# LonglongaaaGo/VSPBFR

Hardware: AMD Instinct MI355X
Metric: restored 512x512 faces/sec (higher is better)
Workload: dtype f32; 1 GPU; restoration_test.py hot path A+B+C+D, batch 8/GPU, 512x512, 50-step DDPM CodeDiffuser + StyleGAN2 prior + RestoreNet forward, fp32, random-init weights; batch_per_gpu=8, with_style_sample=True, sampler=ddpm, overlap=A+B of batch i+1 on a second HIP stream under C+D of batch i, launch=eager (one host launch per kernel)

## Files before the change

### include/vspbfr_hip.h

```cpp
#ifndef VSPBFR_HIP_H
#define VSPBFR_HIP_H

#include <stdint.h>

#ifdef __cplusplus
extern "C" {
#endif

#define VSP_ABI_VERSION 4

#define VSP_OK 0
#define VSP_EINVAL (-1)
#define VSP_ELAUNCH (-2)
#define VSP_ENOTSUP (-3)

typedef void* vsp_stream_t;

int vsp_abi_version(void);
const char* vsp_last_error(void);
int vsp_device_count(void);
int vsp_struct_size(int which);

int vsp_fused_bias_act_f32(float* out, const float* x, const float* bias, const float* ref, int64_t n,
                           int step_b, int size_b, int act, int grad, float alpha, float scale,
// ... 92 lines not shown
  const float* Bm;
  float* C;
  int Z, M, N, K;
  int64_t a_zs, a_ms, a_ks;
  int64_t b_zs, b_ns, b_ks;
  int64_t c_zs, c_ms;
  float alpha;
  const float* bias;
  float bias_scale;
  int act;
  float slope, gain;
  int64_t bias_zs;
} vsp_gemm_params;

int vsp_gemm_f32(const vsp_gemm_params* p, vsp_stream_t stream);

int vsp_pixelnorm_dim1_f32(float* out, const float* x, int Z, int R, int C, float eps, vsp_stream_t stream);
int vsp_layernorm_f32(float* out, const float* x, const float* add, const float* gamma, const float* beta,
                      int rows, int cols, float eps, int post, float slope, float gain, vsp_stream_t stream);
int vsp_softmax_lastdim_f32(float* out, const float* x, int rows, int cols, vsp_stream_t stream);
int vsp_softmax_dim1_f32(float* out, const float* x, int Z, int R, int C, vsp_stream_t stream);
int vsp_film_f32(float* out, const float* h, const float* gamma, const float* beta, int64_t n,
                 vsp_stream_t stream);
int vsp_axpby_idx_f32(float* out, const float* x, const float* y, const float* a, const float* b, int idx,
                      int64_t n, vsp_stream_t stream);
int vsp_demod_f32(float* out, const float* style, const float* wsq, int B, int Cin, int Cout, float wscale,
                  float eps, vsp_stream_t stream);
typedef struct {
  const float* w;
  const float* bias;
  const float* wsq;
  float* mod;
  float* demod;
  int64_t src_off;
  int cin, cout;
  float alpha, bias_scale, wscale2;
  int pad_;
} vsp_style_layer;
int vsp_style_plan_f32(const vsp_style_layer* table, int L, const float* src, int B, int64_t bstride, int K, int max_cin, int max_cout,
                       float eps, vsp_stream_t stream);
int vsp_demod_weight_f32(float* out, float* wsq, const float* style, const float* w, int B, int Cin, int Cout, int K, float wscale,
                         float eps, vsp_stream_t stream);
int vsp_demod_weight_bwd_f32(float* dstyle, float* dw, const float* g, const float* out, const float* style, const float* wsq,
                             const float* w, int B, int Cin, int Cout, int K, float wscale, vsp_stream_t stream);
int vsp_demod_weight_bwd_acc_f32(float* dstyle, float* dw, const float* g, int g_stride, const float* out, const float* style,
                                 const float* wsq, const float* w, int B, int Cin, int Cout, int K, float wscale, int accumulate,
                                 vsp_stream_t stream);
int vsp_avgpool2x2_f32(float* out, const float* x, int64_t planes, int OH, int OW, vsp_stream_t stream);
int vsp_upsample_add_f32(float* out, const float* x, const float* y, int64_t planes, int IH, int IW, int OH,
                         int OW, vsp_stream_t stream);
int vsp_plane_mean_f32(float* out, const float* x, int64_t planes, int hw, vsp_stream_t stream);
int vsp_scale_add_f32(float* out, const float* x, const float* gate, const float* y, int64_t planes, int hw,
                      vsp_stream_t stream);
int vsp_subsample_f32(float* out, const float* x, int64_t planes, int IH, int IW, int s, vsp_stream_t stream);
int vsp_quantize_u8_nhwc(uint8_t* out, const float* x, int B, int C, int H, int W, float lo, float hi,
                         vsp_stream_t stream);
#define VSP_WIN_UNIFORM7 7
#define VSP_WIN_GAUSS11 11
size_t vsp_pair_stats_work_bytes(int B, int H, int W, int C, int window);
int vsp_pair_stats_u8(unsigned long long* sse, double* ssim, const uint8_t* a, const uint8_t* b, int B, int H, int W, int C,
                      int window, void* work, vsp_stream_t stream);
int vsp_resize_bilinear_f32(float* out, const float* x, int64_t planes, int IH, int IW, int OH, int OW, vsp_stream_t stream);
int vsp_e4e_codes_f32(float* out, const float* heads, const float* latent_avg, int B, int T, int D, vsp_stream_t stream);
int vsp_rows_concat_f32(float* out, int B, int T, int nseg, const float* const* src, const int* batch_stride, const int* token_stride,
                        const int* width, const int* flip, vsp_stream_t stream);
int vsp_add3_f32(float* out, const float* a, const float* b, const float* c, int64_t n, vsp_stream_t stream);

int vsp_pointwise_f32(float* y, const float* x, const float* w, const float* in_scale, const float* ch_bias,
                      const float* bias1, int act1, const float* bias2, int act2, const float* res, const float* up_src,
                      const float* up_kernel, int W, int B, int Cin, int Cout, int64_t HW, vsp_stream_t stream);

int vsp_tacc_scores_f32(float* score, const float* P, int ldp, int k_off, const float* eQ, const float* wq,
                        int wq_stride, float tfrac, int B, int n_tok, int dim, vsp_stream_t stream);
int vsp_tacc_chan_attn_f32(float* t, const float* P, int ldp, int q2_off, int v2_off, const float* ek,
                           const float* wk, int wk_stride, float tfrac, int B, int n_tok, int dim,
                           vsp_stream_t stream);
int vsp_tacc_tail_f32(float* y, float* pn, const float* P, int ldp, int k_off, int v_off, const float* eQ,
                      const float* wq , float tfrac, const float* t, const float* gamma,
                      const float* beta, const float* xold, const float* c1, const float* c2, int idx, int B, int n_tok,
                      int dim, vsp_stream_t stream);
int vsp_tacc_head_pre_f32(float* out, const float* e, const float* wcol, int w_stride, const float* ln_w,
                          const float* ln_b, int S, int M, int dim, float t_div, vsp_stream_t stream);

typedef struct vsp_tacc_block {
  const float* wcat;
  const float* eQ;
  const float* ek;
  const float* wq;
  const float* wk;
  const float* gamma;
  const float* beta;
  const float* wcat_frag;
} vsp_tacc_block;

typedef struct vsp_tacc_chain_params {
  int B, n_tok, dim, n_blocks;
  const vsp_tacc_block* blocks;
  float* x;
  float* work;
  size_t work_floats;
  int n_steps;
  const int* step;
  const int* coef_idx;
  const float* c1;
  const float* c2;
  float t_div;
// ... 199 lines not shown
```

### vspbfr_amd/_lib.py

```python
import ctypes as C
import os

import torch

from .photo import FaceAAItem, FaceItem, FaceTile
from .resample import ResampleItem

_HERE = os.path.dirname(os.path.abspath(__file__))
LIB_PATH = os.environ.get("VSPBFR_HIP_LIB", os.path.join(_HERE, "lib", "libvspbfr_hip.so"))



def tune_env(name, default=None):
    if os.environ.get("VSP_TUNE", "0") in ("", "0"):
        return default
    return os.environ.get(name, default)


ABI_VERSION = 4
c_float_p = C.c_void_p


class FirEpilogue(C.Structure):
    _fields_ = [
# ... 51 lines not shown
    ]


class GemmParams(C.Structure):
    _fields_ = [
        ("A", C.c_void_p), ("Bm", C.c_void_p), ("C", C.c_void_p),
        ("Z", C.c_int), ("M", C.c_int), ("N", C.c_int), ("K", C.c_int),
        ("a_zs", C.c_int64), ("a_ms", C.c_int64), ("a_ks", C.c_int64),
        ("b_zs", C.c_int64), ("b_ns", C.c_int64), ("b_ks", C.c_int64),
        ("c_zs", C.c_int64), ("c_ms", C.c_int64),
        ("alpha", C.c_float), ("bias", C.c_void_p), ("bias_scale", C.c_float),
        ("act", C.c_int), ("slope", C.c_float), ("gain", C.c_float), ("bias_zs", C.c_int64),
    ]


class DegradeItem(C.Structure):
    _fields_ = [("tap_off", C.c_int64), ("pix_off", C.c_int64), ("jpg_off", C.c_int64), ("sample", C.c_int64)] + [
        (n, C.c_int32) for n in ("src", "ksize", "dh", "dw", "quality", "flags", "mcu0", "slot")] + [("alpha", C.c_float), ("sigma", C.c_float)]


DEGRADE_HAZE, DEGRADE_GREY = 1, 2
DEGRADE_MAX_KSIZE, DEGRADE_MAX_SIZE, DEGRADE_MAX_ITEMS = 41, 2048, 1024
WIN_UNIFORM7, WIN_GAUSS11 = 7, 11

_i, _i64, _f, _p = C.c_int, C.c_int64, C.c_float, C.c_void_p

SIGNATURES = {
    "vsp_abi_version": [],
    "vsp_device_count": [],
    "vsp_struct_size": [_i],
    "vsp_fused_bias_act_f32": [_p, _p, _p, _p, _i64, _i, _i, _i, _i, _f, _f, _p],
    "vsp_upfirdn2d_f32": [_p, _p, _p] + [_i] * 14 + [C.POINTER(FirEpilogue), _p],
    "vsp_conv2d_f32": [C.POINTER(ConvParams), _p],
    "vsp_conv2d_num_configs": [],
    "vsp_gemm_f32": [C.POINTER(GemmParams), _p],
    "vsp_pixelnorm_dim1_f32": [_p, _p, _i, _i, _i, _f, _p],
    "vsp_layernorm_f32": [_p, _p, _p, _p, _p, _i, _i, _f, _i, _f, _f, _p],
    "vsp_softmax_lastdim_f32": [_p, _p, _i, _i, _p],
    "vsp_softmax_dim1_f32": [_p, _p, _i, _i, _i, _p],
    "vsp_film_f32": [_p, _p, _p, _p, _i64, _p],
    "vsp_axpby_idx_f32": [_p, _p, _p, _p, _p, _i, _i64, _p],
    "vsp_demod_f32": [_p, _p, _p, _i, _i, _i, _f, _f, _p],
    "vsp_style_plan_f32": [_p, _i, _p, _i, _i64, _i, _i, _i, _f, _p],
    "vsp_demod_weight_f32": [_p, _p, _p, _p, _i, _i, _i, _i, _f, _f, _p],
    "vsp_demod_weight_bwd_f32": [_p, _p, _p, _p, _p, _p, _p, _i, _i, _i, _i, _f, _p],
    "vsp_demod_weight_bwd_acc_f32": [_p, _p, _p, _i, _p, _p, _p, _p, _i, _i, _i, _i, _f, _i, _p],
    "vsp_avgpool2x2_f32": [_p, _p, _i64, _i, _i, _p],
    "vsp_upsample_add_f32": [_p, _p, _p, _i64, _i, _i, _i, _i, _p],
    "vsp_e4e_codes_f32": [_p, _p, _p, _i, _i, _i, _p],
    "vsp_rows_concat_f32": [_p, _i, _i, _i, C.POINTER(C.c_void_p), C.POINTER(_i), C.POINTER(_i), C.POINTER(_i), C.POINTER(_i), _p],
    "vsp_resize_bilinear_f32": [_p, _p, _i64, _i, _i, _i, _i, _p],
    "vsp_plane_mean_f32": [_p, _p, _i64, _i, _p],
    "vsp_scale_add_f32": [_p, _p, _p, _p, _i64, _i, _p],
    "vsp_subsample_f32": [_p, _p, _i64, _i, _i, _i, _p],
    "vsp_add3_f32": [_p, _p, _p, _p, _i64, _p],
    "vsp_pointwise_f32": [_p, _p, _p, _p, _p, _p, _i, _p, _i, _p, _p, _p, _i, _i, _i, _i, _i64, _p],
    "vsp_quantize_u8_nhwc": [_p, _p, _i, _i, _i, _i, _f, _f, _p],
    "vsp_tacc_scores_f32": [_p, _p, _i, _i, _p, _p, _i, _f, _i, _i, _i, _p],
    "vsp_tacc_chan_attn_f32": [_p, _p, _i, _i, _i, _p, _p, _i, _f, _i, _i, _i, _p],
    "vsp_tacc_tail_f32": [_p, _p, _p, _i, _i, _i, _p, _p, _f, _p, _p, _p, _p, _p, _p, _i, _i, _i, _i, _p],
    "vsp_tacc_head_pre_f32": [_p, _p, _p, _i, _p, _p, _i, _i, _i, _f, _p],
    "vsp_tacc_chain_f32": [_p, _p],
    "vsp_conv2d_winograd_f32": [_p, _p],
    "vsp_conv2d_bf16": [_p, _p],
    "vsp_conv2d_bf16x3": [_p, _p],
    "vsp_conv2d_bf16rv": [_p, _p],
    "vsp_conv2d_bf16dg": [_p, _p],
    "vsp_affine_sample_f32": [_p, _p, _p, _i, _i, _i, _i, _i, _i, _p],
    "vsp_affine_sample_bwd_f32": [_p, _p, _p, _i, _i, _i, _i, _i, _i, _p],
    "vsp_color_affine_f32": [_p, _p, _p, _p, _i, _i64, _p],
    "vsp_maxpool2d_f32": [_p, _p, _i64, _i, _i, _i, _i, _i, _i, _i, _p],
    "vsp_maxpool2d_bwd_f32": [_p, _p, _p, _i64, _i, _i, _i, _i, _i, _i, _i, _p],
    "vsp_lpips_layer_f32": [_p, _p, _p, _p, _i, _i, _i, _p],
    "vsp_lpips_layer_bwd_f32": [_p, _p, _p, _p, _p, _i, _i, _i, _p],
    "vsp_resize_bilinear_bwd_f32": [_p, _p, _i64, _i, _i, _i, _i, _p],
    "vsp_conv2d_wgrad_f32": [C.POINTER(ConvWgradParams), _p],
    "vsp_plane_dot_f32": [_p, _p, _p, _i64, _i64, _p],
    "vsp_channel_sum_f32": [_p, _p, _i, _i, _i64, _p],
    "vsp_noise_bias_act_f32": [_p, _p, _p, _p, _p, _i, _i, _i64, C.c_float, C.c_float, _p],
    "vsp_noise_dot_f32": [_p, _p, _p, _i, _i, _i64, _p],
    "vsp_smart_tail_bwd_f32": [_p, _p, _p, _p, _p, _p, _p, _p, _p, _i, _i, _i64, C.c_float, C.c_float, _p],
    "vsp_plane_dot_scale_f32": [_p, _p, _p, _p, _i64, _i64, _p],
    "vsp_convert_f32_to_bf16": [_p, _p, _i64, _p],
    "vsp_convert_bf16_to_f32": [_p, _p, _i64, _p],
    "vsp_upfirdn2d_bf16": [_p, _p, _p] + [_i] * 14 + [C.POINTER(FirEpilogue), _p],
    "vsp_pointwise_bf16": [_p, _p, _p, _p, _p, _p, _i, _p, _i, _p, _p, _p, _i, _i, _i, _i, _i64, _p],
    "vsp_keyed_fill_f32": [_p, _i, C.POINTER(C.c_int64), C.POINTER(C.c_int32), _i, C.c_uint64, _i64, _p, _i, _p],
    "vsp_conv1x1_small_f32": [_p, _p, _p, _p, _i, _i, _i, _i, _i, _f, _f, _p],
    "vsp_pack_weight_f32": [_p, _p, _i, _i, _i, _i, _i, _i, _i, _f, _p],
    "vsp_winograd_weight_f32": [_p, _p, _i, _i, _i, _p],
    "vsp_winograd4_weight_f32": [_p, _p, _i, _i, _p],
    "vsp_conv2d_winograd4_f32": [_p, _p, C.c_size_t, _p],
    "vsp_winograd4f_weight_f32": [_p, _p, _i, _i, _p],
    "vsp_conv2d_winograd4f_f32": [_p, _p],
    "vsp_modulate_weight_bf16": [_p, _p, _p, _i, _i64, _i, _i, _i, _p],
    "vsp_conv2d_winograd_chunk": [],
    "vsp_conv2d_winograd_mbw": [_i],
    "vsp_degrade_gt_f32": [_p, _p, _p, _p, _i, _i, _i, _p],
    "vsp_degrade_blur_f32": [_p, _p, _p, _p, _i, _i, _i, _i, _p],
    "vsp_degrade_down_u8": [_p, _p, _p, _p, _p, _i, _i, _i, _i, C.c_uint64, _i64, _p],
    "vsp_degrade_jpeg_u8": [_p, _p, _p, _i, _i, _i, _p],
    "vsp_degrade_up_f32": [_p, _p, _p, _i, _i, _i, _p],
    "vsp_pair_stats_u8": [_p, _p, _p, _p, _i, _i, _i, _i, _i, _p, _p],
    "vsp_lanczos_resize_u8": [_p, _p, _p, C.c_size_t, _p, C.c_size_t, _p, C.c_size_t, _p, _p, _i, _i, _i, _p],
    "vsp_png_encode_u8": [_p, C.c_size_t, _p, _p, _p, _i, _i, _i, _i, _p],
    "vsp_niqe_features_u8": [_p, _p, _p, _p, _i, _i, _i, _i, _p, _p, _p],
# ... 58 lines not shown
```

### vspbfr_amd/csrc/rowops.hip

```cpp
#include "vsp_common.h"

namespace {

__device__ __forceinline__ float wave_sum(float v) {
#pragma unroll
  for (int o = 32; o > 0; o >>= 1) v += __shfl_xor(v, o, 64);
  return v;
}
__device__ __forceinline__ float wave_max(float v) {
#pragma unroll
  for (int o = 32; o > 0; o >>= 1) v = fmaxf(v, __shfl_xor(v, o, 64));
  return v;
}

inline int stream_blocks(int64_t n) {
  int64_t b = (n + 255) / 256;
  if (b > vsp::kMaxStreamBlocks) b = vsp::kMaxStreamBlocks;
  return (int)(b < 1 ? 1 : b);
}

__global__ __launch_bounds__(256) void pixelnorm_dim1_kernel(float* out, const float* x, int Z, int R, int C, float eps) {
  const int64_t total = (int64_t)Z * C;
  for (int64_t i = (int64_t)blockIdx.x * blockDim.x + threadIdx.x; i < total; i += (int64_t)gridDim.x * blockDim.x) {
    const int z = (int)(i / C), c = (int)(i % C);
// ... 202 lines not shown

__global__ __launch_bounds__(256) void upsample_add_kernel(float* out, const float* x, const float* y, int64_t planes, int IH,
                                                            int IW, int OH, int OW, float ry, float rx) {
  const int64_t total = planes * OH * OW;
  for (int64_t i = (int64_t)blockIdx.x * blockDim.x + threadIdx.x; i < total; i += (int64_t)gridDim.x * blockDim.x) {
    const int ox = (int)(i % OW);
    const int64_t t = i / OW;
    const int oy = (int)(t % OH);
    const int64_t pl = t / OH;
    const float fy = ry * (float)oy, fx = rx * (float)ox;
    int y0 = (int)fy, x0 = (int)fx;
    if (y0 > IH - 1) y0 = IH - 1;
    if (x0 > IW - 1) x0 = IW - 1;
    const int y1 = y0 + (y0 < IH - 1 ? 1 : 0), x1 = x0 + (x0 < IW - 1 ? 1 : 0);
    const float ly = fy - (float)y0, lx = fx - (float)x0;
    const float hy = 1.f - ly, hx = 1.f - lx;
    const float* xp = x + pl * IH * IW;
    const float v = hy * (hx * xp[y0 * IW + x0] + lx * xp[y0 * IW + x1]) + ly * (hx * xp[y1 * IW + x0] + lx * xp[y1 * IW + x1]);
    out[i] = v + y[i];
  }
}

__global__ __launch_bounds__(256) void resize_bilinear_kernel(float* out, const float* x, int64_t planes, int IH, int IW, int OH,
                                                               int OW, float sy, float sx) {
  const int64_t total = planes * OH * OW;
  for (int64_t i = (int64_t)blockIdx.x * blockDim.x + threadIdx.x; i < total; i += (int64_t)gridDim.x * blockDim.x) {
    const int ox = (int)(i % OW);
    const int64_t t = i / OW;
    const int oy = (int)(t % OH);
    const int64_t pl = t / OH;
    const float fy = fmaxf(((float)oy + 0.5f) * sy - 0.5f, 0.f), fx = fmaxf(((float)ox + 0.5f) * sx - 0.5f, 0.f);
    int y0 = (int)fy, x0 = (int)fx;
    if (y0 > IH - 1) y0 = IH - 1;
    if (x0 > IW - 1) x0 = IW - 1;
    const int y1 = y0 + (y0 < IH - 1 ? 1 : 0), x1 = x0 + (x0 < IW - 1 ? 1 : 0);
    const float ly = fy - (float)y0, lx = fx - (float)x0;
    const float hy = 1.f - ly, hx = 1.f - lx;
    const float* xp = x + pl * IH * IW;
    out[i] = hy * (hx * xp[y0 * IW + x0] + lx * xp[y0 * IW + x1]) + ly * (hx * xp[y1 * IW + x0] + lx * xp[y1 * IW + x1]);
  }
}

__global__ __launch_bounds__(256) void plane_mean_kernel(float* out, const float* x, int64_t planes, int hw) {
  const int lane = threadIdx.x & 63;
  const int64_t pl = (int64_t)blockIdx.x * 4 + (threadIdx.x >> 6);
  if (pl >= planes) return;
  const float* xp = x + pl * hw;
  float s = 0.f;
  for (int i = lane; i < hw; i += 64) s += xp[i];
  s = wave_sum(s);
  if (lane == 0) out[pl] = s / (float)hw;
}

__global__ __launch_bounds__(256) void scale_add_kernel(float* out, const float* x, const float* gate, const float* y, int64_t planes,
                                                         int hw) {
  const int64_t total = planes * hw;
  for (int64_t i = (int64_t)blockIdx.x * blockDim.x + threadIdx.x; i < total; i += (int64_t)gridDim.x * blockDim.x) {
    const float g = gate[i / hw];
    out[i] = x[i] * g + (y ? y[i] : 0.f);
  }
}

__global__ __launch_bounds__(256) void subsample_kernel(float* out, const float* x, int64_t planes, int IH, int IW, int OH, int OW,
                                                         int s) {
  const int64_t total = planes * OH * OW;
  for (int64_t i = (int64_t)blockIdx.x * blockDim.x + threadIdx.x; i < total; i += (int64_t)gridDim.x * blockDim.x) {
    const int ox = (int)(i % OW);
    const int64_t t = i / OW;
    const int oy = (int)(t % OH);
    const int64_t pl = t / OH;
    out[i] = x[(pl * IH + (int64_t)oy * s) * IW + (int64_t)ox * s];
  }
}

__global__ __launch_bounds__(256) void quantize_u8_nhwc_kernel(uint8_t* out, const float* x, int B, int C, int H, int W, float lo,
                                                               float hi, float range) {
  const int64_t total = (int64_t)B * H * W * C;
  for (int64_t i = (int64_t)blockIdx.x * blockDim.x + threadIdx.x; i < total; i += (int64_t)gridDim.x * blockDim.x) {
    const int c = (int)(i % C);
    int64_t t = i / C;
    const int xw = (int)(t % W);
    t /= W;
    const int y = (int)(t % H);
    const int b = (int)(t / H);
    float v = x[(((int64_t)b * C + c) * H + y) * W + xw];
    v = fminf(fmaxf(v, lo), hi);
    v = (v - lo) / range;
    v = fminf(fmaxf(v * 255.f + 0.5f, 0.f), 255.f);
    out[i] = (uint8_t)v;
  }
}

__global__ __launch_bounds__(256) void add3_kernel(float* out, const float* a, const float* b, const float* c, int64_t n) {
  for (int64_t i = (int64_t)blockIdx.x * blockDim.x + threadIdx.x; i < n; i += (int64_t)gridDim.x * blockDim.x)
    out[i] = a[i] + b[i] + (c ? c[i] : 0.f);
}

}

__global__ __launch_bounds__(256) void e4e_codes_kernel(float* __restrict__ out, const float* __restrict__ heads,
                                                         const float* __restrict__ avg, int B, int T, int D) {
  const int64_t total = (int64_t)B * T * D;
  for (int64_t i = (int64_t)blockIdx.x * blockDim.x + threadIdx.x; i < total; i += (int64_t)gridDim.x * blockDim.x) {
    const int j = (int)(i % D);
    const int64_t r = i / D;
    const int t = (int)(r % T), b = (int)(r / T);
    float v = heads[((int64_t)t * B + b) * D + j];
    if (t > 0) v += heads[(int64_t)b * D + j];
    if (avg) v += avg[t * D + j];
    out[i] = v;
  }
}

struct ConcatSeg {
  const float* src;
  int bs, ts, width, flip;
};
struct ConcatArgs {
  ConcatSeg seg[3];
  int nseg, B, T, W;
};

__global__ __launch_bounds__(256) void rows_concat_kernel(float* __restrict__ out, ConcatArgs a) {
  const int64_t total = (int64_t)a.B * a.T * a.W;
// ... 105 lines not shown
  VSP_REQUIRE(B >= 0 && Cin >= 1 && Cout >= 1 && K >= 1, "demod_weight_bwd: bad dims");
  VSP_REQUIRE(g && out && style && (!dstyle || wsq) && (!dw || w), "demod_weight_bwd: null pointer");
  VSP_REQUIRE(B <= 65535 && g_stride >= Cout, "demod_weight_bwd: batch too large / gradient row pitch below Cout");
  const float c = -0.5f * wscale * wscale;
  hipStream_t st = vsp::as_stream(stream);
  if (dw) {
    const int64_t n = (int64_t)Cout * Cin;
    demod_weight_bwd_w_kernel<<<(unsigned)((n + 255) / 256), 256, 0, st>>>(dw, g, g_stride, out, style, w, B, Cin, Cout, K, c, accumulate ? 1 : 0);
  }
  if (dstyle && B > 0) {
    const size_t lds = (size_t)(Cout + 256) * sizeof(float);
    VSP_REQUIRE(lds <= 64 * 1024, "demod_weight_bwd: too many output channels (%d)", Cout);
    demod_weight_bwd_s_kernel<<<dim3((unsigned)((Cin + 63) / 64), (unsigned)B), 256, lds, st>>>(dstyle, g, g_stride, out, style, wsq, Cin, Cout, c,
                                                                                                   accumulate ? 1 : 0);
  }
  return vsp::check_launch("demod_weight_bwd");
}

int vsp_avgpool2x2_f32(float* out, const float* x, int64_t planes, int OH, int OW, vsp_stream_t stream) {
  VSP_REQUIRE(planes >= 0 && OH >= 0 && OW >= 0, "avgpool2x2: bad dims");
  const int64_t n = planes * OH * OW;
  if (n == 0) return VSP_OK;
  VSP_REQUIRE(out && x, "avgpool2x2: null pointer");
  VSP_REQUIRE((reinterpret_cast<uintptr_t>(x) & 7u) == 0, "avgpool2x2: input must be 8-byte aligned");
  VSP_LAUNCH_1D(avgpool2x2_kernel, n, stream, out, x, planes, OH, OW);
  return vsp::check_launch("avgpool2x2");
}

int vsp_upsample_add_f32(float* out, const float* x, const float* y, int64_t planes, int IH, int IW, int OH, int OW,
                         vsp_stream_t stream) {
  VSP_REQUIRE(planes >= 0 && IH >= 1 && IW >= 1 && OH >= 1 && OW >= 1, "upsample_add: bad dims");
  const int64_t n = planes * OH * OW;
  if (n == 0) return VSP_OK;
  VSP_REQUIRE(out && x && y, "upsample_add: null pointer");
  const float ry = OH > 1 ? (float)(IH - 1) / (float)(OH - 1) : 0.f;
  const float rx = OW > 1 ? (float)(IW - 1) / (float)(OW - 1) : 0.f;
  VSP_LAUNCH_1D(upsample_add_kernel, n, stream, out, x, y, planes, IH, IW, OH, OW, ry, rx);
  return vsp::check_launch("upsample_add");
}

int vsp_resize_bilinear_f32(float* out, const float* x, int64_t planes, int IH, int IW, int OH, int OW, vsp_stream_t stream) {
  VSP_REQUIRE(planes >= 0 && IH >= 1 && IW >= 1 && OH >= 1 && OW >= 1, "resize_bilinear: bad dims");
  const int64_t n = planes * OH * OW;
  if (n == 0) return VSP_OK;
  VSP_REQUIRE(out && x, "resize_bilinear: null pointer");
  VSP_LAUNCH_1D(resize_bilinear_kernel, n, stream, out, x, planes, IH, IW, OH, OW, (float)IH / (float)OH, (float)IW / (float)OW);
  return vsp::check_launch("resize_bilinear");
}

int vsp_plane_mean_f32(float* out, const float* x, int64_t planes, int hw, vsp_stream_t stream) {
  VSP_REQUIRE(planes >= 0 && hw >= 1, "plane_mean: bad dims");
  if (planes == 0) return VSP_OK;
  VSP_REQUIRE(out && x, "plane_mean: null pointer");
  plane_mean_kernel<<<(unsigned)((planes + 3) / 4), 256, 0, vsp::as_stream(stream)>>>(out, x, planes, hw);
  return vsp::check_launch("plane_mean");
}

int vsp_scale_add_f32(float* out, const float* x, const float* gate, const float* y, int64_t planes, int hw,
                      vsp_stream_t stream) {
  VSP_REQUIRE(planes >= 0 && hw >= 1, "scale_add: bad dims");
  if (planes == 0) return VSP_OK;
  VSP_REQUIRE(out && x && gate, "scale_add: null pointer");
  VSP_LAUNCH_1D(scale_add_kernel, planes * hw, stream, out, x, gate, y, planes, hw);
  return vsp::check_launch("scale_add");
}

int vsp_subsample_f32(float* out, const float* x, int64_t planes, int IH, int IW, int s, vsp_stream_t stream) {
  VSP_REQUIRE(planes >= 0 && IH >= 1 && IW >= 1 && s >= 1, "subsample: bad dims");
  const int OH = (IH - 1) / s + 1, OW = (IW - 1) / s + 1;
  if (planes == 0) return VSP_OK;
  VSP_REQUIRE(out && x, "subsample: null pointer");
  VSP_LAUNCH_1D(subsample_kernel, planes * OH * OW, stream, out, x, planes, IH, IW, OH, OW, s);
  return vsp::check_launch("subsample");
}

int vsp_quantize_u8_nhwc(uint8_t* out, const float* x, int B, int C, int H, int W, float lo, float hi, vsp_stream_t stream) {
  VSP_REQUIRE(B >= 0 && C >= 1 && H >= 0 && W >= 0, "quantize_u8: bad dims");
  const int64_t n = (int64_t)B * C * H * W;
  if (n == 0) return VSP_OK;
  VSP_REQUIRE(out && x, "quantize_u8: null pointer");
  const float range = hi - lo > 1e-5f ? hi - lo : 1e-5f;
  VSP_LAUNCH_1D(quantize_u8_nhwc_kernel, n, stream, out, x, B, C, H, W, lo, hi, range);
  return vsp::check_launch("quantize_u8_nhwc");
}

int vsp_e4e_codes_f32(float* out, const float* heads, const float* latent_avg, int B, int T, int D, vsp_stream_t stream) {
  VSP_REQUIRE(B >= 0 && T >= 1 && D >= 1, "e4e_codes: bad dims");
  if (B == 0) return VSP_OK;
  VSP_REQUIRE(out && heads, "e4e_codes: null pointer");
  VSP_LAUNCH_1D(e4e_codes_kernel, (int64_t)B * T * D, stream, out, heads, latent_avg, B, T, D);
  return vsp::check_launch("e4e_codes");
}

int vsp_rows_concat_f32(float* out, int B, int T, int nseg, const float* const* src, const int* batch_stride, const int* token_stride,
                        const int* width, const int* flip, vsp_stream_t stream) {
  VSP_REQUIRE(B >= 0 && T >= 1 && nseg >= 1 && nseg <= 3, "rows_concat: 1..3 segments");
  if (B == 0) return VSP_OK;
  VSP_REQUIRE(out && src && batch_stride && token_stride && width && flip, "rows_concat: null pointer");
  ConcatArgs a{};
  a.nseg = nseg; a.B = B; a.T = T; a.W = 0;
  for (int k = 0; k < nseg; ++k) {
    VSP_REQUIRE(src[k] && width[k] >= 1, "rows_concat: bad segment %d", k);
    a.seg[k] = ConcatSeg{src[k], batch_stride[k], token_stride[k], width[k], flip[k]};
    a.W += width[k];
  }
  VSP_LAUNCH_1D(rows_concat_kernel, (int64_t)B * T * a.W, stream, out, a);
  return vsp::check_launch("rows_concat");
}

int vsp_add3_f32(float* out, const float* a, const float* b, const float* c, int64_t n, vsp_stream_t stream) {
  if (n <= 0) return VSP_OK;
  VSP_REQUIRE(out && a && b, "add3: null pointer");
  VSP_LAUNCH_1D(add3_kernel, n, stream, out, a, b, c, n);
  return vsp::check_launch("add3");
}

}
```

### vspbfr_amd/e4e.py

```python
import math
from argparse import Namespace

import torch
from torch import nn

from . import hip_ops as H
from .layers import EqualLinear, NoiseInjection, PixelNorm, StyledConv, ToRGB, _Cached, style_context

IR50_BLOCKS = ((64, 64, 3), (64, 128, 4), (128, 256, 14), (256, 512, 3))


class ConstantInput(nn.Module):
    def __init__(self, channel, size=4):
        super().__init__()
        self.input = nn.Parameter(torch.randn(1, channel, size, size))

    def forward(self, batch):
        stamp = (self.input.data_ptr(), self.input._version, self.input.device, batch)
        hit = self.__dict__.get("_rep")
        if hit is None or hit[0] != stamp:
            hit = (stamp, self.input.detach().repeat(batch, 1, 1, 1))
            self.__dict__["_rep"] = hit
        return hit[1]

# ... 78 lines not shown
    return a.contiguous(), (bn.bias - bn.running_mean * a).contiguous()


def _plain_pack(conv):
    w = conv.weight
    return H.PackedConv(H.pack_weight(w.contiguous()), 1, w.shape[0], w.shape[1], w.shape[2], w.shape[3], conv.stride[0],
                        (1,), (conv.padding[0],))


class SEModule(nn.Module):
    def __init__(self, channels, reduction):
        super().__init__()
        self.fc1 = nn.Conv2d(channels, channels // reduction, kernel_size=1, padding=0, bias=False)
        self.fc2 = nn.Conv2d(channels // reduction, channels, kernel_size=1, padding=0, bias=False)

    def gate(self, x):
        m = H.plane_mean(x)
        h = H.gemm_nt(m, self.fc1.weight.view(self.fc1.weight.shape[0], -1), act=1, slope=0.0, gain=1.0)
        return H.gemm_nt(h, self.fc2.weight.view(self.fc2.weight.shape[0], -1), act=2)


class bottleneck_IR_SE(_Cached):

    def __init__(self, in_channel, depth, stride):
        super().__init__()
        self.stride, self.same = stride, in_channel == depth
        if self.same:
            self.shortcut_layer = nn.MaxPool2d(1, stride)
        else:
            self.shortcut_layer = nn.Sequential(nn.Conv2d(in_channel, depth, (1, 1), stride, bias=False), nn.BatchNorm2d(depth))
        self.res_layer = nn.Sequential(
            nn.BatchNorm2d(in_channel), nn.Conv2d(in_channel, depth, (3, 3), (1, 1), 1, bias=False), nn.PReLU(depth),
            nn.Conv2d(depth, depth, (3, 3), stride, 1, bias=False), nn.BatchNorm2d(depth), SEModule(depth, 16))

    def _consts(self):
        r = self.res_layer
        src = [r[0].weight, r[0].bias, r[0].running_mean, r[0].running_var, r[1].weight, r[3].weight, r[4].weight, r[4].bias,
               r[4].running_mean, r[4].running_var]
        if not self.same:
            s = self.shortcut_layer
            src += [s[0].weight, s[1].weight, s[1].bias, s[1].running_mean, s[1].running_var]

        def build():
            d = {"bn0": _bn_fold(r[0]), "c1": _plain_pack(r[1]), "c2": _plain_pack(r[3]), "bn4": _bn_fold(r[4])}
            if not self.same:
                d["sc"] = _plain_pack(self.shortcut_layer[0])
                d["scbn"] = _bn_fold(self.shortcut_layer[1])
            return d
        return self._derive("consts", src, build)

    def forward(self, x):
        c = self._consts()
        r = self.res_layer
        if self.same:
            shortcut = x if self.stride == 1 else H.subsample(x, self.stride)
        else:
            shortcut = H.conv2d_packed(x, c["sc"], ch_scale=c["scbn"][0], ch_bias=c["scbn"][1])
        y = H.conv2d_packed(x, c["c1"], in_scale=c["bn0"][0], in_scale_per_sample=False, in_shift=c["bn0"][1], act2=2,
                            prelu=r[2].weight)
        y = H.conv2d_packed(y, c["c2"], ch_scale=c["bn4"][0], ch_bias=c["bn4"][1])
        return H.scale_add(y, r[5].gate(y), shortcut)


class GradualStyleBlock(_Cached):

    def __init__(self, in_c, out_c, spatial):
        super().__init__()
        self.out_c, self.spatial = out_c, spatial
        mods = []
        c = in_c
        for _ in range(int(math.log2(spatial))):
            mods += [nn.Conv2d(c, out_c, kernel_size=3, stride=2, padding=1), nn.LeakyReLU()]
            c = out_c
        self.convs = nn.Sequential(*mods)
        self.linear = EqualLinear(out_c, out_c, lr_mul=1)

    def forward(self, x):
        convs = [m for m in self.convs if isinstance(m, nn.Conv2d)]
        packs = self._derive("packs", [m.weight for m in convs], lambda: [_plain_pack(m) for m in convs])
        for m, pc in zip(convs, packs):
            x = H.conv2d_packed(x, pc, ch_bias=m.bias, act2=1, slope2=0.01, gain2=1.0)
        return self.linear(x.view(-1, self.out_c))


class Encoder4Editing(_Cached):
    def __init__(self, num_layers, mode="ir", opts=None):
        super().__init__()
        assert num_layers == 50 and mode == "ir_se", "the restoration path uses the IR-SE50 backbone only"
        in_ch = getattr(opts, "input_channel", 3)
        self.input_layer = nn.Sequential(nn.Conv2d(in_ch, 64, (3, 3), 1, 1, bias=False), nn.BatchNorm2d(64), nn.PReLU(64))
        units = []
        for in_c, depth, n in IR50_BLOCKS:
            units.append(bottleneck_IR_SE(in_c, depth, 2))
            units += [bottleneck_IR_SE(depth, depth, 1) for _ in range(n - 1)]
        self.body = nn.Sequential(*units)
        log_size = int(math.log(opts.stylegan_size, 2))
        self.style_count = 2 * log_size - 2
        self.coarse_ind, self.middle_ind = 3, 7
        self.styles = nn.ModuleList(
            GradualStyleBlock(512, 512, 16 if i < self.coarse_ind else 32 if i < self.middle_ind else 64)
            for i in range(self.style_count))
        self.latlayer1 = nn.Conv2d(256, 512, kernel_size=1, stride=1, padding=0)
        self.latlayer2 = nn.Conv2d(128, 512, kernel_size=1, stride=1, padding=0)

    @torch.no_grad()
    def forward(self, x, latent_avg=None):
        il = self.input_layer
        src = [il[0].weight, il[1].weight, il[1].bias, il[1].running_mean, il[1].running_var, self.latlayer1.weight,
               self.latlayer2.weight]
        c = self._derive("consts", src, lambda: {"in": _plain_pack(il[0]), "bn": _bn_fold(il[1]),
                                                 "l1": _plain_pack(self.latlayer1), "l2": _plain_pack(self.latlayer2)})
        x = H.conv2d_packed(x.contiguous(), c["in"], ch_scale=c["bn"][0], ch_bias=c["bn"][1], act2=2, prelu=il[2].weight)
        taps = {}
# ... 184 lines not shown
```

### vspbfr_amd/hip_ops.py

```python
import ctypes as C
import math
from collections import namedtuple

import os

import torch

from . import _lib
from ._lib import ConvParams, FirEpilogue, GemmParams, check, lib, tune_env

SQRT2 = math.sqrt(2.0)


class ConvProfiler:

    def __init__(self):
        self.records = []

    def begin(self):
        ev = torch.cuda.Event(enable_timing=True)
        ev.record()
        return ev

    def end(self, start, flops, tag, nbytes=0):
# ... 979 lines not shown
def maxpool2d(x, k, s, p=0):
    x = _req(x, "x")
    B, Cc, H, W = x.shape
    OH, OW = (H + 2 * p - k) // s + 1, (W + 2 * p - k) // s + 1
    out = torch.empty((B, Cc, OH, OW), device=x.device, dtype=x.dtype)
    check(lib.vsp_maxpool2d_f32(_ptr(out), _ptr(x), B * Cc, H, W, OH, OW, k, s, p, _stream()), "maxpool2d")
    return out


def maxpool2d_bwd(dy, x, k, s, p=0):
    x, dy = _req(x, "x"), _req(dy, "dy")
    B, Cc, H, W = x.shape
    OH, OW = dy.shape[-2:]
    dx = torch.empty_like(x)
    check(lib.vsp_maxpool2d_bwd_f32(_ptr(dx), _ptr(dy), _ptr(x), B * Cc, H, W, OH, OW, k, s, p, _stream()), "maxpool2d_bwd")
    return dx


def lpips_layer(f0, f1, w):
    f0, f1, w = _req(f0, "f0"), _req(f1, "f1"), _req(w, "w")
    B, Cc, H, W = f0.shape
    if f1.shape != f0.shape or w.numel() != Cc:
        raise RuntimeError("lpips_layer: f0 / f1 / w shapes do not match")
    out = torch.empty((B,), device=f0.device, dtype=torch.float32)
    check(lib.vsp_lpips_layer_f32(_ptr(out), _ptr(f0), _ptr(f1), _ptr(w), B, Cc, H * W, _stream()), "lpips_layer")
    return out


def lpips_layer_bwd(gout, f0, f1, w):
    f0, f1, w, gout = _req(f0, "f0"), _req(f1, "f1"), _req(w, "w"), _req(gout, "gout")
    B, Cc, H, W = f0.shape
    df1 = torch.empty_like(f1)
    check(lib.vsp_lpips_layer_bwd_f32(_ptr(df1), _ptr(f0), _ptr(f1), _ptr(w), _ptr(gout), B, Cc, H * W, _stream()), "lpips_layer_bwd")
    return df1


def plane_mean(x):
    x = _req(x, "x")
    B, Cc, H, W = x.shape
    out = torch.empty((B, Cc), device=x.device, dtype=x.dtype)
    check(lib.vsp_plane_mean_f32(_ptr(out), _ptr(x), B * Cc, H * W, _stream()), "plane_mean")
    return out


def scale_add(x, gate, y=None):
    x = _req(x, "x")
    B, Cc, H, W = x.shape
    out = torch.empty_like(x)
    check(lib.vsp_scale_add_f32(_ptr(out), _ptr(x), _ptr(_req(gate, "gate")), _ptr(_opt(y, "y")), B * Cc, H * W,
                                _stream()), "scale_add")
    return out


def subsample(x, s):
    x = _req(x, "x")
    B, Cc, H, W = x.shape
    out = torch.empty((B, Cc, (H - 1) // s + 1, (W - 1) // s + 1), device=x.device, dtype=x.dtype)
    check(lib.vsp_subsample_f32(_ptr(out), _ptr(x), B * Cc, H, W, s, _stream()), "subsample")
    return out


def add3(a, b, c=None):
    out = torch.empty_like(_req(a, "a"))
    check(lib.vsp_add3_f32(_ptr(out), _ptr(a), _ptr(_req(b, "b")), _ptr(_opt(c, "c")), a.numel(), _stream()), "add3")
    return out


def tacc_scores(P, eQ, wq_col, tfrac, B, k_off=0):
    score = torch.empty((B, 18, 18), device=P.device, dtype=P.dtype)
    check(lib.vsp_tacc_scores_f32(_ptr(score), _ptr(_req(P, "P")), P.shape[1], k_off, _ptr(_req(eQ, "eQ")),
                                  C.c_void_p(wq_col.data_ptr()), wq_col.stride(0), float(tfrac), B, 18, 512, _stream()),
          "tacc_scores")
    return score


def tacc_chan_attn(P, ek, wk_col, tfrac, B, q2_off=1024, v2_off=1536):
    t = torch.empty((B, 18, 512), device=P.device, dtype=P.dtype)
    check(lib.vsp_tacc_chan_attn_f32(_ptr(t), _ptr(_req(P, "P")), P.shape[1], q2_off, v2_off, _ptr(_req(ek, "ek")),
                                     C.c_void_p(wk_col.data_ptr()), wk_col.stride(0), float(tfrac), B, 18, 512, _stream()),
          "tacc_chan_attn")
    return t


def tacc_tail(P, eQ, wq, tfrac, t, gamma, beta, B, xold=None, c1=None, c2=None, idx=0, k_off=0, v_off=512, want_pn=True):
    y = torch.empty((B, 18, 512), device=P.device, dtype=P.dtype)
    pn = torch.empty_like(y) if want_pn else None
    check(lib.vsp_tacc_tail_f32(_ptr(y), _ptr(pn), _ptr(_req(P, "P")), P.shape[1], k_off, v_off, _ptr(_req(eQ, "eQ")),
                                _ptr(_req(wq, "wq")), float(tfrac), _ptr(_req(t, "t")), _ptr(_req(gamma, "gamma")),
                                _ptr(_req(beta, "beta")), _ptr(_opt(xold, "xold")), _ptr(_opt(c1, "c1")), _ptr(_opt(c2, "c2")),
                                int(idx), B, 18, 512, _stream()), "tacc_tail")
    return y, pn


def tacc_head_pre(e, wcol, ln_w, ln_b, steps, t_div):
    M = e.shape[0]
    out = torch.empty((steps * M, 512), device=e.device, dtype=e.dtype)
    check(lib.vsp_tacc_head_pre_f32(_ptr(out), _ptr(_req(e, "e")), C.c_void_p(wcol.data_ptr()), wcol.stride(0),
                                    _ptr(_req(ln_w, "ln_w")), _ptr(_req(ln_b, "ln_b")), steps, M, 512, float(t_div), _stream()),
          "tacc_head_pre")
    return out


def pointwise(x, w, in_scale=None, ch_bias=None, bias1=None, bias2=None, res=None, up_src=None, up_kernel=None):
    x = _req(x, "x", bf16_ok=True)
    B, Cin, Hh, Ww = x.shape
    Cout = w.shape[0]
# ... 470 lines not shown
```

Measured before the change: 205.6 img/s.

## Fuse SE gate MLP, sigmoid, scale and shortcut add into one kernel

In inference mode, the bottleneck-IR block tail now uses a single kernel. It computes the SE squeeze MLP (fc1, ReLU, fc2, sigmoid) per block from the plane means, then writes y*gate + shortcut, reading a strided shortcut directly so the separate subsample launch is dropped. This removes several small launches and intermediate tensors in an eager-launch setting. The SE MLP is recomputed redundantly in every block, and plane_mean gains a one-workgroup-per-plane variant for large planes.

```diff
diff --git a/include/vspbfr_hip.h b/include/vspbfr_hip.h
--- a/include/vspbfr_hip.h
+++ b/include/vspbfr_hip.h
@@ -168,6 +168,9 @@
 int vsp_plane_mean_f32(float* out, const float* x, int64_t planes, int hw, vsp_stream_t stream);
 int vsp_scale_add_f32(float* out, const float* x, const float* gate, const float* y, int64_t planes, int hw,
                       vsp_stream_t stream);
+int vsp_se_tail_f32(float* out, const float* y, const float* mean, const float* fc1, const float* fc2, int hidden, const float* sc,
+                    int64_t sc_bs, int64_t sc_cs, int64_t sc_hs, int64_t sc_ws, int SH, int SW, int step, int B, int C, int H, int W,
+                    vsp_stream_t stream);
 int vsp_subsample_f32(float* out, const float* x, int64_t planes, int IH, int IW, int s, vsp_stream_t stream);
 int vsp_quantize_u8_nhwc(uint8_t* out, const float* x, int B, int C, int H, int W, float lo, float hi,
                          vsp_stream_t stream);
diff --git a/vspbfr_amd/_lib.py b/vspbfr_amd/_lib.py
--- a/vspbfr_amd/_lib.py
+++ b/vspbfr_amd/_lib.py
@@ -127,6 +127,7 @@
     "vsp_resize_bilinear_f32": [_p, _p, _i64, _i, _i, _i, _i, _p],
     "vsp_plane_mean_f32": [_p, _p, _i64, _i, _p],
     "vsp_scale_add_f32": [_p, _p, _p, _p, _i64, _i, _p],
+    "vsp_se_tail_f32": [_p, _p, _p, _p, _p, _i, _p, _i64, _i64, _i64, _i64, _i, _i, _i, _i, _i, _i, _i, _p],
     "vsp_subsample_f32": [_p, _p, _i64, _i, _i, _i, _p],
     "vsp_add3_f32": [_p, _p, _p, _p, _i64, _p],
     "vsp_pointwise_f32": [_p, _p, _p, _p, _p, _p, _i, _p, _i, _p, _p, _p, _i, _i, _i, _i, _i64, _p],
diff --git a/vspbfr_amd/csrc/rowops.hip b/vspbfr_amd/csrc/rowops.hip
--- a/vspbfr_amd/csrc/rowops.hip
+++ b/vspbfr_amd/csrc/rowops.hip
@@ -278,6 +278,30 @@
   if (lane == 0) out[pl] = s / (float)hw;
 }
 
+constexpr int kPlaneWg = 4096;
+template <bool VEC>
+__global__ __launch_bounds__(256) void plane_mean_wg_kernel(float* out, const float* x, int hw) {
+  __shared__ float part[4];
+  const float* xp = x + (int64_t)blockIdx.x * hw;
+  float s = 0.f;
+  if (VEC) {
+    float4 a = make_float4(0.f, 0.f, 0.f, 0.f);
+#pragma unroll 4
+    for (int i = threadIdx.x * 4; i < hw; i += 1024) {
+      const float4 v = *reinterpret_cast<const float4*>(xp + i);
+      a.x += v.x, a.y += v.y, a.z += v.z, a.w += v.w;
+    }
+    s = (a.x + a.y) + (a.z + a.w);
+  } else {
+#pragma unroll 4
+    for (int i = threadIdx.x; i < hw; i += 256) s += xp[i];
+  }
+  s = wave_sum(s);
+  if ((threadIdx.x & 63) == 0) part[threadIdx.x >> 6] = s;
+  __syncthreads();
+  if (threadIdx.x == 0) out[blockIdx.x] = ((part[0] + part[1]) + (part[2] + part[3])) / (float)hw;
+}
+
 __global__ __launch_bounds__(256) void scale_add_kernel(float* out, const float* x, const float* gate, const float* y, int64_t planes,
                                                          int hw) {
   const int64_t total = planes * hw;
@@ -296,6 +320,96 @@
     const int oy = (int)(t % OH);
     const int64_t pl = t / OH;
     out[i] = x[(pl * IH + (int64_t)oy * s) * IW + (int64_t)ox * s];
+  }
+}
+
+constexpr int kSeCG = 16;
+constexpr int kSeMaxC = 2048;
+constexpr int kSeChunk = 4096;
+
+struct SeTail {
+  float* out;
+  const float *y, *mean, *fc1, *fc2, *sc;
+  int64_t sc_bs, sc_cs, sc_hs, sc_ws;
+  int C, R, H, W;
+};
+
+template <bool VEC, bool SCVEC>
+__global__ __launch_bounds__(256) void se_tail_kernel(const SeTail p) {
+  __shared__ float m_s[kSeMaxC];
+  __shared__ float h_s[kSeMaxC / 16];
+  __shared__ float g_s[kSeCG];
+  const int tid = threadIdx.x, lane = tid & 63, wave = tid >> 6;
+  const int b = blockIdx.z, c0 = blockIdx.y * kSeCG;
+  const int hw = p.H * p.W, n = kSeCG * hw;
+  const int e0 = blockIdx.x * kSeChunk;
+  const int64_t base = ((int64_t)b * p.C + c0) * hw;
+  const float* scb = p.sc + b * p.sc_bs + c0 * p.sc_cs;
+  auto sc_at = [&](int e) {
+    const int cl = e / hw, pix = e - cl * hw;
+    const int oy = pix / p.W, ox = pix - oy * p.W;
+    return scb + cl * p.sc_cs + oy * p.sc_hs + ox * p.sc_ws;
+  };
+
+  constexpr int NV = kSeChunk / 1024;
+  float4 yv[NV], sv[NV];
+  if (VEC) {
+#pragma unroll
+    for (int i = 0; i < NV; ++i) {
+      const int e = e0 + i * 1024 + tid * 4;
+      if (e < n) {
+        yv[i] = *reinterpret_cast<const float4*>(p.y + base + e);
+        const float* sp = sc_at(e);
+        if (SCVEC) sv[i] = *reinterpret_cast<const float4*>(sp);
+        else sv[i] = make_float4(sp[0], sp[p.sc_ws], sp[2 * p.sc_ws], sp[3 * p.sc_ws]);
+      }
+    }
+  }
+
+  for (int c = tid; c < p.C; c += 256) m_s[c] = p.mean[(int64_t)b * p.C + c];
+  __syncthreads();
+  for (int j0 = wave * 4; j0 < p.R; j0 += 16) {
+    const float* w1[4];
+#pragma unroll
+    for (int u = 0; u < 4; ++u) w1[u] = p.fc1 + (int64_t)min(j0 + u, p.R - 1) * p.C;
+    float a[4] = {0.f, 0.f, 0.f, 0.f};
+#pragma unroll 4
+    for (int c = lane; c < p.C; c += 64) {
+      const float mv = m_s[c];
+#pragma unroll
+      for (int u = 0; u < 4; ++u) a[u] = fmaf(w1[u][c], mv, a[u]);
+    }
+#pragma unroll
+    for (int u = 0; u < 4; ++u) {
+      a[u] = wave_sum(a[u]);
+      if (lane == 0 && j0 + u < p.R) h_s[j0 + u] = fmaxf(a[u], 0.f);
+    }
+  }
+  __syncthreads();
+  {
+    const int cl = tid >> 4, s = tid & 15;
+    const float* w2 = p.fc2 + (int64_t)(c0 + cl) * p.R;
+    float a = 0.f;
+    for (int j = s; j < p.R; j += 16) a = fmaf(w2[j], h_s[j], a);
+#pragma unroll
+    for (int o = 8; o > 0; o >>= 1) a += __shfl_xor(a, o, 64);
+    if (s == 0) g_s[cl] = 1.f / (1.f + expf(-a));
+  }
+  __syncthreads();
+
+  if (VEC) {
+#pragma unroll
+    for (int i = 0; i < NV; ++i) {
+      const int e = e0 + i * 1024 + tid * 4;
+      if (e < n) {
+        const float g = g_s[e / hw];
+        *reinterpret_cast<float4*>(p.out + base + e) =
+            make_float4(fmaf(yv[i].x, g, sv[i].x), fmaf(yv[i].y, g, sv[i].y), fmaf(yv[i].z, g, sv[i].z), fmaf(yv[i].w, g, sv[i].w));
+      }
+    }
+  } else {
+    const int e1 = min(e0 + kSeChunk, n);
+    for (int e = e0 + tid; e < e1; e += 256) p.out[base + e] = fmaf(p.y[base + e], g_s[e / hw], *sc_at(e));
   }
 }
 
@@ -507,7 +621,12 @@
   VSP_REQUIRE(planes >= 0 && hw >= 1, "plane_mean: bad dims");
   if (planes == 0) return VSP_OK;
   VSP_REQUIRE(out && x, "plane_mean: null pointer");
-  plane_mean_kernel<<<(unsigned)((planes + 3) / 4), 256, 0, vsp::as_stream(stream)>>>(out, x, planes, hw);
+  if (hw >= kPlaneWg && planes <= 0x7fffffff) {
+    if (hw % 4 == 0 && vsp::aligned16(x)) plane_mean_wg_kernel<true><<<(unsigned)planes, 256, 0, vsp::as_stream(stream)>>>(out, x, hw);
+    else plane_mean_wg_kernel<false><<<(unsigned)planes, 256, 0, vsp::as_stream(stream)>>>(out, x, hw);
+  } else {
+    plane_mean_kernel<<<(unsigned)((planes + 3) / 4), 256, 0, vsp::as_stream(stream)>>>(out, x, planes, hw);
+  }
   return vsp::check_launch("plane_mean");
 }
 
@@ -527,6 +646,27 @@
   VSP_REQUIRE(out && x, "subsample: null pointer");
   VSP_LAUNCH_1D(subsample_kernel, planes * OH * OW, stream, out, x, planes, IH, IW, OH, OW, s);
   return vsp::check_launch("subsample");
+}
+
+int vsp_se_tail_f32(float* out, const float* y, const float* mean, const float* fc1, const float* fc2, int hidden, const float* sc,
+                    int64_t sc_bs, int64_t sc_cs, int64_t sc_hs, int64_t sc_ws, int SH, int SW, int step, int B, int C, int H, int W,
+                    vsp_stream_t stream) {
+  VSP_REQUIRE(B >= 1 && B <= 65535 && C >= 1 && H >= 1 && W >= 1 && (int64_t)H * W <= (1 << 26), "se_tail: bad dims");
+  VSP_REQUIRE(C % 16 == 0 && C <= kSeMaxC, "se_tail: C must be a multiple of 16, at most %d (got %d)", kSeMaxC, C);
+  VSP_REQUIRE(hidden * 16 == C, "se_tail: fc1 / fc2 have %d hidden units, C / 16 = %d", hidden, C / 16);
+  VSP_REQUIRE(step >= 1 && SH >= 1 && SW >= 1 && (SH - 1) / step + 1 == H && (SW - 1) / step + 1 == W,
+              "se_tail: a %d x %d shortcut read at step %d does not give the %d x %d map", SH, SW, step, H, W);
+  VSP_REQUIRE(sc_bs >= 0 && sc_cs >= 0 && sc_hs >= 0 && sc_ws >= 0, "se_tail: negative shortcut stride");
+  VSP_REQUIRE(out && y && mean && fc1 && fc2 && sc, "se_tail: null pointer");
+  SeTail p{out, y, mean, fc1, fc2, sc, sc_bs, sc_cs, sc_hs * step, sc_ws * step, C, hidden, H, W};
+  const dim3 grid((unsigned)((kSeCG * H * W + kSeChunk - 1) / kSeChunk), (unsigned)(C / kSeCG), (unsigned)B);
+  hipStream_t st = vsp::as_stream(stream);
+  const bool vec = W % 4 == 0 && vsp::aligned16(out) && vsp::aligned16(y);
+  const bool scvec = vec && p.sc_ws == 1 && vsp::aligned16(sc) && p.sc_bs % 4 == 0 && p.sc_cs % 4 == 0 && p.sc_hs % 4 == 0;
+  if (scvec) se_tail_kernel<true, true><<<grid, 256, 0, st>>>(p);
+  else if (vec) se_tail_kernel<true, false><<<grid, 256, 0, st>>>(p);
+  else se_tail_kernel<false, false><<<grid, 256, 0, st>>>(p);
+  return vsp::check_launch("se_tail");
 }
 
 int vsp_quantize_u8_nhwc(uint8_t* out, const float* x, int B, int C, int H, int W, float lo, float hi, vsp_stream_t stream) {
diff --git a/vspbfr_amd/e4e.py b/vspbfr_amd/e4e.py
--- a/vspbfr_amd/e4e.py
+++ b/vspbfr_amd/e4e.py
@@ -154,13 +154,18 @@
     def forward(self, x):
         c = self._consts()
         r = self.res_layer
+        fused = not torch.is_grad_enabled()
         if self.same:
-            shortcut = x if self.stride == 1 else H.subsample(x, self.stride)
+            shortcut = x if self.stride == 1 or fused else H.subsample(x, self.stride)
         else:
             shortcut = H.conv2d_packed(x, c["sc"], ch_scale=c["scbn"][0], ch_bias=c["scbn"][1])
         y = H.conv2d_packed(x, c["c1"], in_scale=c["bn0"][0], in_scale_per_sample=False, in_shift=c["bn0"][1], act2=2,
                             prelu=r[2].weight)
         y = H.conv2d_packed(y, c["c2"], ch_scale=c["bn4"][0], ch_bias=c["bn4"][1])
+        if fused:
+            se = r[5]
+            return H.se_tail(y, H.plane_mean(y), se.fc1.weight.view(se.fc1.weight.shape[0], -1),
+                             se.fc2.weight.view(se.fc2.weight.shape[0], -1), shortcut, self.stride if self.same else 1)
         return H.scale_add(y, r[5].gate(y), shortcut)
 
 
diff --git a/vspbfr_amd/hip_ops.py b/vspbfr_amd/hip_ops.py
--- a/vspbfr_amd/hip_ops.py
+++ b/vspbfr_amd/hip_ops.py
@@ -1055,6 +1055,21 @@
     return out
 
 
+def se_tail(y, mean, fc1, fc2, shortcut, step=1):
+    y, mean, fc1, fc2 = _req(y, "y"), _req(mean, "mean"), _req(fc1, "fc1"), _req(fc2, "fc2")
+    B, Cc, H, W = y.shape
+    if not (isinstance(shortcut, torch.Tensor) and shortcut.is_cuda and shortcut.dtype == torch.float32 and shortcut.dim() == 4):
+        raise RuntimeError("se_tail: shortcut must be a 4-d float32 CUDA tensor")
+    hidden = fc1.shape[0]
+    if (tuple(mean.shape) != (B, Cc) or tuple(fc1.shape) != (hidden, Cc) or tuple(fc2.shape) != (Cc, hidden)
+            or tuple(shortcut.shape[:2]) != (B, Cc)):
+        raise RuntimeError("se_tail: y / mean / fc1 / fc2 / shortcut shapes do not match")
+    out = torch.empty_like(y)
+    check(lib.vsp_se_tail_f32(_ptr(out), _ptr(y), _ptr(mean), _ptr(fc1), _ptr(fc2), hidden, _ptr(shortcut), *shortcut.stride(),
+                              shortcut.shape[2], shortcut.shape[3], int(step), B, Cc, H, W, _stream()), "se_tail")
+    return out
+
+
 def subsample(x, s):
     x = _req(x, "x")
     B, Cc, H, W = x.shape
```

Measured after the change: 207.4 img/s (median of 6 runs). Within noise of the previous version (+0.9%).
